# mburger-stsci/nexoclom

Hardware: AMD Instinct MI355X
Metric: particle*steps/s (higher is better)
Workload: dtype f64

## Files before the change

nexoclom_amd/csrc/nxc_device.hpp:

```cpp
#pragma once
#include <hip/hip_runtime.h>
#include <stdint.h>
#include "nxc_math.hpp"

struct LutDesc {
    int rec, fs, cell;
    int top;
    int last;
    int pad_;
    double xbase;
    double inv_w;
};
typedef LutDesc LutView;

extern __shared__ __align__(32) unsigned char nxc_lds[];

#define NXC_LDS_AS __attribute__((address_space(3)))
#define NXC_GLOBAL_AS __attribute__((address_space(1)))
typedef double nxc_v2d __attribute__((ext_vector_type(2)));

NXC_DEV double lds_f64(int byte_off)
{
    return *(const NXC_LDS_AS double *)(unsigned)byte_off;
}
// ... 491 lines not shown
    const double rn = nxc_sqrt((x * x + y * y) + z * z);
    const double en = nxc_sqrt(y * y + x * x);
    const double n0 = -z * x, n1 = -z * y, n2 = x * x + y * y;
    const double nn = nxc_sqrt((n0 * n0 + n1 * n1) + n2 * n2);
    const double dx = (v_t0 * (n0 / nn) + v_t1 * (y / en)) + v_rad * (x / rn);
    const double dy = (v_t0 * (n1 / nn) + v_t1 * (-x / en)) + v_rad * (y / rn);
    const double dz = (v_t0 * (n2 / nn) + v_t1 * 0.0) + v_rad * (z / rn);
    const double lonhit = fmod(atan2(x, -y) + TWO_PI, TWO_PI);
    const double lathit = asin(z);
    double tsurf = B.t0;
    if (lonhit <= 1.5707963267948966 || lonhit >= 4.71238898038469)
        tsurf = B.t0 + B.t1 * nxc_sqrt(nxc_sqrt(__builtin_fabs(cos(lonhit) * cos(lathit))));
    double v_new;
    if (B.accom == 0.0) {
        v_new = nxc_sqrt(v_old2);
    } else {
        const double v_emit = bispev3(B, tsurf, u_p) / B.unit_km;
        v_new = nxc_sqrt(v_emit * v_emit * B.accom + v_old2 * (1 - B.accom));
    }
    const double wx = dx * v_new, wy = dy * v_new, wz = dz * v_new;
    double frac = s[7];
    if (B.temp_dependent == 2) {
        double st = stick_map_at(B, lonhit, lathit);
        st = st > 1. ? 1. : (st < 0. ? 0. : st);
        frac *= (1 - st);
    } else if (B.temp_dependent) {
        double st = B.A0 * exp(B.A1 * tsurf) + B.A2;
        st = st > 1. ? 1. : (st < 0. ? 0. : st);
        frac *= (1 - st);
    } else if (B.stickcoef > 0) {
        frac *= (1 - B.stickcoef);
    }
    const double zero = ((x * 0.0 + y * 0.0) + (z * 0.0 + frac * 0.0)) + ((wx * 0.0 + wy * 0.0) + wz * 0.0);
    if (zero != 0.0) return false;
    s[1] = x; s[2] = y; s[3] = z;
    s[4] = wx; s[5] = wy; s[6] = wz;
    s[7] = frac;
    return true;
}

template <bool BOUNCE, bool NBODY = false>
NXC_DEV void apply_fate(double (&s)[8], double edge2, unsigned long long id, int &nbounce,
                        unsigned long long &nonfinite, const BodyK *Bd = nullptr,
                        const double *__restrict__ base = nullptr)
{
    const double r2 = (s[1] * s[1] + s[2] * s[2]) + s[3] * s[3];
    if (r2 < 1.0) {
        if (BOUNCE) {
            if (!bounce_packet(lds_header().B, s, r2, id, nbounce)) { s[7] = 0.0; nonfinite++; }
        } else s[7] = 0.0;
    }
    if (r2 > edge2) s[7] = 0.0;
    if (NBODY) {
        for (int m = 0; m < Bd->n_moons; m++) {
            double mx, my;
            moon_position(*Bd, base, m, 5, mx, my);
            const double dx = s[1] - mx, dy = s[2] - my;
            if ((dx * dx + dy * dy) + s[3] * s[3] < Bd->rad2[m]) s[7] = 0.0;
        }
    }
    if (s[7] < 1e-10) s[7] = 0.0;
    if (s[7] == 0.0) s[0] = 0.0;
}


NXC_DEV double wave_uniform(double v)
{
    const long long b = __double_as_longlong(v);
    const int lo = __builtin_amdgcn_readfirstlane((int)(b & 0xffffffffll));
    const int hi = __builtin_amdgcn_readfirstlane((int)(b >> 32));
    return __longlong_as_double(((long long)hi << 32) | (unsigned int)lo);
}
NXC_DEV int wave_uniform(int v) { return __builtin_amdgcn_readfirstlane(v); }

struct ImageRegs {
    double vrplanet;
    double x_lo, x_hi, x_inv_step, z_lo, z_hi, z_inv_step;
    int xedges, zedges, nx, nz, quantity, n_lines, downcast, dbg, x_is_x;
};

NXC_DEV ImageRegs image_regs(const ImageK &G)
{
    ImageRegs R;
    R.vrplanet = G.vrplanet;
    R.xedges = (int)G.xedges_off; R.zedges = (int)G.zedges_off;
    R.nx = G.nx; R.nz = G.nz;
    R.x_lo = lds_f64(R.xedges); R.x_hi = lds_f64(R.xedges + 8 * R.nx);
    R.z_lo = lds_f64(R.zedges); R.z_hi = lds_f64(R.zedges + 8 * R.nz);
    R.x_inv_step = G.x_inv_step; R.z_inv_step = G.z_inv_step;
    R.quantity = G.quantity; R.n_lines = G.n_lines; R.downcast = G.downcast_f32;
    R.x_is_x = wave_uniform(G.x_is_x);
#ifdef NXC_EXPERIMENT_KNOBS
    R.dbg = G.dbg;
#else
    R.dbg = 0;
#endif
    R.vrplanet = wave_uniform(R.vrplanet);
    R.x_lo = wave_uniform(R.x_lo); R.x_hi = wave_uniform(R.x_hi);
    R.z_lo = wave_uniform(R.z_lo); R.z_hi = wave_uniform(R.z_hi);
    R.x_inv_step = wave_uniform(R.x_inv_step); R.z_inv_step = wave_uniform(R.z_inv_step);
    R.xedges = wave_uniform(R.xedges); R.zedges = wave_uniform(R.zedges);
    R.nx = wave_uniform(R.nx); R.nz = wave_uniform(R.nz);
    R.quantity = wave_uniform(R.quantity); R.n_lines = wave_uniform(R.n_lines);
    R.downcast = wave_uniform(R.downcast);
#ifdef NXC_EXPERIMENT_KNOBS
    R.dbg = wave_uniform(R.dbg);
#endif
    return R;
}

NXC_DEV double nxc_div_const(double n, double d, double y)
{
    if (!((nxc_mid_range(n) || n == 0.0) && y == y)) return n / d;
    return nxc_div_seeded(n, d, y);
}

NXC_DEV int bin_index(double v, int edges, int n, double lo, double hi, double inv_step)
{
    if (!(v >= lo) || !(v <= hi)) return -1;
    int k = (int)((v - lo) * inv_step);
    k = k > n - 1 ? n - 1 : k;
    const double e0 = lds_f64(edges + 8 * k), e1 = lds_f64(edges + 8 * k + 8);
    if (__builtin_expect(!((v >= e0) && (v < e1)), 0)) {
        while (k > 0 && v < lds_f64(edges + 8 * k)) --k;
        while (k < n - 1 && v >= lds_f64(edges + 8 * (k + 1))) ++k;
    }
    return k;
}

NXC_DEV double f32_round_trip(double v) { return (double)(float)v; }

NXC_DEV int half_swap(int v, bool upper)
{
    const auto r = __builtin_amdgcn_permlane32_swap(v, v, false, false);
    return upper ? (int)r[0] : (int)r[1];
}

NXC_DEV void image_add_pairs(bool has, int pix, double w, double *__restrict__ acc2)
{
    if (__ballot(has) == 0) return;
    const bool upper = (threadIdx.x & 32) != 0;
    const int ppix = half_swap(has ? pix : -1, upper);
    const bool own = has && w != 0.0;
    const bool partner = ppix >= 0;
    {
        const bool act = upper ? partner : own;
        if (act)
            unsafeAtomicAdd(&acc2[2ll * (upper ? ppix : pix) + (upper ? 1 : 0)], upper ? 1.0 : w);
    }
    {
        const bool act = upper ? own : partner;
        if (act)
            unsafeAtomicAdd(&acc2[2ll * (upper ? pix : ppix) + (upper ? 0 : 1)], upper ? w : 1.0);
    }
}

NXC_DEV bool image_locate_core_xz(const ImageK &G, const ImageRegs &R, double x, double y, double z,
                                  double vy, double frac, double &radvel_out, double &fw_out,
                                  unsigned long long &nonfinite, int &ix_out, int &iz_out)
{
    const double radvel = vy + R.vrplanet;
    double xo, yo, zo;
    if (R.x_is_x) {
        xo = x;
        yo = G.M[4] * y + G.M[5] * z;
        zo = G.M[7] * y + G.M[8] * z;
    } else {
        xo = (G.M[0] * x + G.M[1] * y) + G.M[2] * z;
        yo = (G.M[3] * x + G.M[4] * y) + G.M[5] * z;
        zo = (G.M[6] * x + G.M[7] * y) + G.M[8] * z;
    }
    const int ix = bin_index(xo, R.xedges, R.nx, R.x_lo, R.x_hi, R.x_inv_step);
    const int iz = bin_index(zo, R.zedges, R.nz, R.z_lo, R.z_hi, R.z_inv_step);
    if (ix < 0 || iz < 0) {
        if (!(__builtin_fabs(frac) <= 1.7976931348623157e308) || radvel != radvel) nonfinite++;
        return false;
    }
    const double s_obs = xo * xo + zo * zo;
    const bool inview = (s_obs > 0x1.0000000000001p+0) || (yo < 0.0);
    frac = inview ? frac : frac * 0.0;
    if (R.quantity != 0)
        frac = sunlit(x, y, z) ? frac : frac * 0.0;
    radvel_out = radvel;
    fw_out = frac;
    ix_out = ix; iz_out = iz;
    return true;
}

NXC_DEV int image_locate_core(const ImageK &G, const ImageRegs &R, double x, double y, double z,
                              double vy, double frac, double &radvel_out, double &fw_out,
                              unsigned long long &nonfinite)
{
    int ix = 0, iz = 0;
    if (!image_locate_core_xz(G, R, x, y, z, vy, frac, radvel_out, fw_out, nonfinite, ix, iz))
        return -1;
    return ix * R.nz + iz;
}

NXC_DEV int image_locate(const ImageK &G, const ImageRegs &R, double x, double y, double z,
                         double vy, double frac, double &radvel_out, double &fw_out,
                         unsigned long long &nonfinite)
{
    if (R.downcast) {
        x = f32_round_trip(x); y = f32_round_trip(y); z = f32_round_trip(z);
        vy = f32_round_trip(vy); frac = f32_round_trip(frac);
    }
    return image_locate_core(G, R, x, y, z, vy, frac, radvel_out, fw_out, nonfinite);
}

NXC_DEV bool image_frame_test(const ImageK &G, const ImageRegs &R, double x, double y, double z,
                              double vy, double frac, float &xf, float &yf, float &zf,
                              unsigned long long &nonfinite)
{
    xf = (float)x; yf = (float)y; zf = (float)z;
    const double xd = xf, yd = yf, zd = zf;
    double xo, zo;
    if (R.x_is_x) {
        xo = xd;
        zo = G.M[7] * yd + G.M[8] * zd;
    } else {
        xo = (G.M[0] * xd + G.M[1] * yd) + G.M[2] * zd;
        zo = (G.M[6] * xd + G.M[7] * yd) + G.M[8] * zd;
    }
    const bool inside = (xo >= R.x_lo) && (xo <= R.x_hi) && (zo >= R.z_lo) && (zo <= R.z_hi);
    if (!inside && (!(__builtin_fabs(frac) < 0x1.ffffffp127) || vy != vy)) nonfinite++;
    return inside;
}

NXC_DEV bool image_weight(const ImageK &G, const ImageRegs &R, double radvel, double fw,
                          double &w_out)
{
    double w = fw;
    if (R.quantity != 0) {
        double gg = 0.0;
        if (R.n_lines == 2) {
            const LutView v0 = lut_view(G.line[0]), v1 = lut_view(G.line[1]);
            LutProbe p0, p1;
            lut_probe_cell(v0, radvel, p0); lut_probe_cell(v1, radvel, p1);
            lut_probe_rows(v0, p0); lut_probe_rows(v1, p1);
            const double g0 = lut_finish(v0, p0);
            gg = g0 + lut_finish(v1, p1);
        } else {
            gg = R.n_lines > 0 ? lut_interp(lut_view(G.line[0]), radvel) : 0.0;
#pragma unroll
            for (int l = 1; l < 4; l++)
                if (l < R.n_lines) gg += lut_interp(lut_view(G.line[l]), radvel);
        }
        w = nxc_div_const(fw * gg, 1e6, lds_header().Wt.rs_1e6);
    }
    w = nxc_div_const(w, G.apix_cm2, lds_header().Wt.rs_apix);
    w_out = w;
    return (__builtin_fabs(w) <= 1.7976931348623157e308) && radvel == radvel;
}

NXC_DEV void image_sample(const ImageK &G, const ImageRegs &R, bool has, double x, double y,
                          double z, double vy, double frac, double *__restrict__ acc2,
                          unsigned long long &binned, unsigned long long &nonfinite)
{
    int pix = -1;
    double radvel = 0.0, fw = 0.0, w = 0.0;
    if (has) pix = image_locate(G, R, x, y, z, vy, frac, radvel, fw, nonfinite);
    bool ok = pix >= 0;
    if (ok && !image_weight(G, R, radvel, fw, w)) { nonfinite++; ok = false; }
    binned += ok;
    image_add_pairs(ok, pix, w, acc2);
}

constexpr int NXC_IMGQ_SLOTS = 128;
constexpr int NXC_IMGQ_BYTES = NXC_IMGQ_SLOTS * (8 + 8 + 4);

struct ImageQueue {
    int head = 0, tail = 0;

    NXC_DEV void push(bool has, int pix, double radvel, double fw, int qoff)
    {
        const unsigned long long m = __ballot(has);
        if (m == 0) return;
        if (has) {
            const int lane = threadIdx.x & 63;
            const int slot = (tail + __popcll(m & ((1ull << lane) - 1ull))) & (NXC_IMGQ_SLOTS - 1);
            *reinterpret_cast<double *>(nxc_lds + qoff + 8 * slot) = radvel;
            *reinterpret_cast<double *>(nxc_lds + qoff + 8 * NXC_IMGQ_SLOTS + 8 * slot) = fw;
            *reinterpret_cast<int *>(nxc_lds + qoff + 16 * NXC_IMGQ_SLOTS + 4 * slot) = pix;
        }
        tail += __popcll(m);
        __builtin_amdgcn_fence(__ATOMIC_RELEASE, "wavefront");
        __builtin_amdgcn_wave_barrier();
    }
    NXC_DEV void push_sample(bool has, float x, float y, float z, float vy, float frac, int qoff)
    {
        const unsigned long long m = __ballot(has);
        if (m == 0) return;
        if (has) {
            const int lane = threadIdx.x & 63;
            const int slot = (tail + __popcll(m & ((1ull << lane) - 1ull))) & (NXC_IMGQ_SLOTS - 1);
            float *q = reinterpret_cast<float *>(nxc_lds + qoff) + slot;
            q[0] = x; q[NXC_IMGQ_SLOTS] = y; q[2 * NXC_IMGQ_SLOTS] = z;
            q[3 * NXC_IMGQ_SLOTS] = vy; q[4 * NXC_IMGQ_SLOTS] = frac;
        }
        tail += __popcll(m);
        __builtin_amdgcn_fence(__ATOMIC_RELEASE, "wavefront");
        __builtin_amdgcn_wave_barrier();
    }
    NXC_DEV bool pop_sample(int qoff, double &x, double &y, double &z, double &vy, double &frac)
    {
        __builtin_amdgcn_fence(__ATOMIC_ACQUIRE, "wavefront");
        const int n = waiting() < 64 ? waiting() : 64;
        const int lane = threadIdx.x & 63;
        const bool mine = lane < n;
        if (mine) {
            const int slot = (head + lane) & (NXC_IMGQ_SLOTS - 1);
            const float *q = reinterpret_cast<const float *>(nxc_lds + qoff) + slot;
            x = q[0]; y = q[NXC_IMGQ_SLOTS]; z = q[2 * NXC_IMGQ_SLOTS];
            vy = q[3 * NXC_IMGQ_SLOTS]; frac = q[4 * NXC_IMGQ_SLOTS];
        }
        head += n;
        __builtin_amdgcn_wave_barrier();
        return mine;
    }
    NXC_DEV int waiting() const { return tail - head; }
    NXC_DEV bool pop(int qoff, int &pix, double &radvel, double &fw)
    {
        __builtin_amdgcn_fence(__ATOMIC_ACQUIRE, "wavefront");
        const int n = waiting() < 64 ? waiting() : 64;
        const int lane = threadIdx.x & 63;
        const bool mine = lane < n;
        if (mine) {
            const int slot = (head + lane) & (NXC_IMGQ_SLOTS - 1);
            radvel = *reinterpret_cast<const double *>(nxc_lds + qoff + 8 * slot);
            fw = *reinterpret_cast<const double *>(nxc_lds + qoff + 8 * NXC_IMGQ_SLOTS + 8 * slot);
            pix = *reinterpret_cast<const int *>(nxc_lds + qoff + 16 * NXC_IMGQ_SLOTS + 4 * slot);
        }
        head += n;
        __builtin_amdgcn_wave_barrier();
        return mine;
    }
};
```

nexoclom_amd/csrc/nxc_kernels.hpp:

```cpp
#pragma once
#include "nxc_device.hpp"

struct DevCounters {
    unsigned long long particle_steps, samples, samples_binned, nonfinite, bad_step, neg_frac,
        unfinished, queue_head;
    unsigned long long wave_trips;
#ifdef NXC_STAMPS
    unsigned long long stamp[8];
#endif
};

#ifdef NXC_STAMPS
NXC_DEV unsigned long long nxc_stamp()
{
    unsigned long long t;
    __builtin_amdgcn_sched_barrier(0);
    asm volatile("s_memtime %0\n\ts_waitcnt lgkmcnt(0)" : "=s"(t) : : "memory");
    __builtin_amdgcn_sched_barrier(0);
    return t;
}
#define NXC_STAMP(k) do { const unsigned long long t_ = nxc_stamp(); seg[k] += t_ - t_prev; t_prev = t_; } while (0)
#else
#define NXC_STAMP(k) do { } while (0)
#endif

constexpr int NXC_BLOCK = 256;
#ifndef NXC_BLOCK_PERSIST_N
#define NXC_BLOCK_PERSIST_N 768
#endif
#ifndef NXC_CHUNK_N
#define NXC_CHUNK_N 32
#endif
constexpr int NXC_BLOCK_PERSIST = NXC_BLOCK_PERSIST_N;
constexpr int NXC_CHUNK = NXC_CHUNK_N;
static_assert(NXC_CHUNK >= 1 && NXC_CHUNK <= 64, "a chunk is loaded by one wave");
constexpr int NXC_WAVE_STAGE_BYTES = NXC_CHUNK * 9 * 8;
constexpr int NXC_WAVE_LDS_BYTES = NXC_WAVE_STAGE_BYTES + NXC_IMGQ_BYTES;
constexpr int NXC_WAVE_LDS_BYTES_ROWS = NXC_CHUNK * 11 * 8;

NXC_DEV void stage_tables(const unsigned char *__restrict__ blob, int64_t bytes)
{
    if ((unsigned)(size_t)(NXC_LDS_AS unsigned char *)nxc_lds != 0u) __builtin_trap();
    const unsigned long long *src = reinterpret_cast<const unsigned long long *>(blob);
    unsigned long long *dst = reinterpret_cast<unsigned long long *>(nxc_lds);
    const int64_t words = bytes >> 3;
    for (int64_t w = threadIdx.x; w < words; w += blockDim.x) dst[w] = src[w];
    __syncthreads();
    if (threadIdx.x == 0) {
        LdsHeader &H = lds_header_rw();
        H.Wt.rs_1e6 = nxc_recip_seed(1e6);
        H.Wt.rs_apix = nxc_mid_range(H.G.apix_cm2) ? nxc_recip_seed(H.G.apix_cm2)
                                                   : __builtin_nan("");
    }
    __syncthreads();
}

NXC_DEV void stage_tables_and_args(const unsigned char *__restrict__ blob, int64_t bytes,
                                   const double *soa0, const unsigned *order, double *final_out,
                                   long long *steps_out, unsigned long long *head, long long n,
                                   const long long *offsets = nullptr,
                                   const unsigned long long *avail = nullptr)
{
    stage_tables(blob, bytes);
    if (threadIdx.x == 0) {
        LoopK &L = lds_header_rw().L;
        L.soa0 = soa0; L.order = order; L.final_out = final_out; L.steps_out = steps_out;
        L.head = head; L.n = n; L.offsets = offsets; L.avail = avail;
        L.q_rec = order ? 8 : 1; L.q_col = order ? 1 : n;
    }
    __syncthreads();
}

NXC_DEV unsigned long long wave_sum(unsigned long long v)
{
#pragma unroll
    for (int off = 32; off > 0; off >>= 1) v += __shfl_down(v, off, 64);
    return v;
}

NXC_DEV void flush_counter(unsigned long long *dst, unsigned long long v)
{
    v = wave_sum(v);
    if ((threadIdx.x & 63) == 0 && v) atomicAdd(dst, v);
}

NXC_DEV void flush_counters_wg(unsigned long long *lds, unsigned long long *d0, unsigned long long v0,
                               unsigned long long *d1, unsigned long long v1,
                               unsigned long long *d2, unsigned long long v2)
{
    __syncthreads();
    if (threadIdx.x < 3) lds[threadIdx.x] = 0ull;
    __syncthreads();
    v0 = wave_sum(v0); v1 = wave_sum(v1); v2 = wave_sum(v2);
    if ((threadIdx.x & 63) == 0) {
        if (v0) atomicAdd(&lds[0], v0);
        if (v1) atomicAdd(&lds[1], v1);
        if (v2) atomicAdd(&lds[2], v2);
    }
    __syncthreads();
    if (threadIdx.x == 0) {
        if (lds[0]) atomicAdd(d0, lds[0]);
        if (lds[1]) atomicAdd(d1, lds[1]);
        if (lds[2]) atomicAdd(d2, lds[2]);
    }
}

NXC_DEV long long wave_bcast0(long long v)
{
    int lo = __builtin_amdgcn_readfirstlane((int)(v & 0xffffffffll));
    int hi = __builtin_amdgcn_readfirstlane((int)(v >> 32));
    return ((long long)hi << 32) | (unsigned int)lo;
}

__global__ void __launch_bounds__(NXC_BLOCK)
k_state(ForceK F, const unsigned char *__restrict__ blob, int64_t stage_bytes, int64_t n,
        const double *__restrict__ x, const double *__restrict__ y, const double *__restrict__ z,
        const double *__restrict__ vy, double *__restrict__ ax, double *__restrict__ ay,
        double *__restrict__ az, double *__restrict__ ion)
{
    stage_tables(blob, stage_bytes);
    const LutView T = lut_view(F.tab);
    for (int64_t i = (int64_t)blockIdx.x * blockDim.x + threadIdx.x; i < n;
         i += (int64_t)gridDim.x * blockDim.x) {
        double a0, a1, a2, l;
        state_eval<false>(F, T, x[i], y[i], z[i], vy[i], a0, a1, a2, l);
        ax[i] = a0; ay[i] = a1; az[i] = a2; ion[i] = l;
    }
}

template <bool DELTA>
__global__ void __launch_bounds__(NXC_BLOCK)
k_rk5_step(ForceK F, const unsigned char *__restrict__ blob, int64_t stage_bytes, int64_t n,
           const double *__restrict__ in, const double *__restrict__ hstep,
           double *__restrict__ out, double *__restrict__ delta)
{
    stage_tables(blob, stage_bytes);
    const LutView T = lut_view(F.tab);
    for (int64_t i = (int64_t)blockIdx.x * blockDim.x + threadIdx.x; i < n;
         i += (int64_t)gridDim.x * blockDim.x) {
        double s[8], d[8];
#pragma unroll
        for (int c = 0; c < 8; c++) s[c] = in[c * n + i];
        rk5_step<DELTA, false>(F, T, s, hstep[i], StepW{}, d);
#pragma unroll
        for (int c = 0; c < 8; c++) out[c * n + i] = s[c];
        if (DELTA) {
#pragma unroll
            for (int c = 0; c < 8; c++) delta[c * n + i] = d[c];
        }
    }
}

constexpr int NXC_REC_DOUBLES = 10;
constexpr int NXC_REC_FLOATS = 10;
typedef float nxc_v4f __attribute__((ext_vector_type(4)));
typedef float nxc_v2f __attribute__((ext_vector_type(2)));
typedef float nxc_v4f_a8 __attribute__((ext_vector_type(4), aligned(8)));

template <int ROWS>
NXC_DEV void store_record(void *__restrict__ rec, long long row, const double (&s)[8],
                          double lossfrac, long long id)
{
    if (ROWS == 2) {
        float *p = static_cast<float *>(rec) + row * NXC_REC_FLOATS;
        nxc_v4f a, b;
        nxc_v2f c;
        a.x = (float)s[0]; a.y = (float)s[1]; a.z = (float)s[2]; a.w = (float)s[3];
        b.x = (float)s[4]; b.y = (float)s[5]; b.z = (float)s[6]; b.w = (float)s[7];
        c.x = (float)lossfrac; c.y = __int_as_float((int)id);
        *reinterpret_cast<nxc_v4f_a8 *>(p) = a;
        *reinterpret_cast<nxc_v4f_a8 *>(p + 4) = b;
        *reinterpret_cast<nxc_v2f *>(p + 8) = c;
    } else {
        nxc_v2d *p = reinterpret_cast<nxc_v2d *>(static_cast<double *>(rec) + row * NXC_REC_DOUBLES);
        nxc_v2d a, b, c, d, e;
        a.x = s[0]; a.y = s[1]; b.x = s[2]; b.y = s[3]; c.x = s[4]; c.y = s[5]; d.x = s[6]; d.y = s[7];
        e.x = lossfrac; e.y = __longlong_as_double(id);
        p[0] = a; p[1] = b; p[2] = c; p[3] = d; p[4] = e;
    }
}

constexpr int NXC_TR_ROWS = 256;
template <typename T, typename I>
__global__ void __launch_bounds__(NXC_TR_ROWS)
k_rows_transpose(const void *__restrict__ rec_, long long total, T *__restrict__ cols,
                 I *__restrict__ index)
{
    static_assert(sizeof(T) == sizeof(I), "a record is ten equal-sized slots");
    typedef T pair_t __attribute__((ext_vector_type(2)));
    __shared__ pair_t tile[NXC_TR_ROWS * 5];
    const T *rec = static_cast<const T *>(rec_);
    for (long long base = (long long)blockIdx.x * NXC_TR_ROWS; base < total;
         base += (long long)gridDim.x * NXC_TR_ROWS) {
        const int nrow = (int)((total - base) < NXC_TR_ROWS ? (total - base) : NXC_TR_ROWS);
        const pair_t *src = reinterpret_cast<const pair_t *>(rec + base * 10);
        for (int w = threadIdx.x; w < nrow * 5; w += NXC_TR_ROWS) tile[w] = src[w];
        __syncthreads();
        if ((int)threadIdx.x < nrow) {
            const T *r = reinterpret_cast<const T *>(tile) + threadIdx.x * 10;
            const long long row = base + threadIdx.x;
#pragma unroll
            for (int c = 0; c < 9; c++) cols[c * total + row] = r[c];
            I id;
            __builtin_memcpy(&id, &r[9], sizeof id);
            index[row] = id;
        }
        __syncthreads();
    }
}

constexpr int NXC_DENSIFY_RECORDS = 32;
__global__ void __launch_bounds__(NXC_BLOCK)
k_rows_densify(const double *__restrict__ rec, const long long *__restrict__ offsets,
               const double *__restrict__ final_soa, const long long *__restrict__ steps,
               int64_t n, int64_t nrec, double *__restrict__ traj)
{
    const int64_t i = (int64_t)blockIdx.x * blockDim.x + threadIdx.x;
    if (i >= n) return;
    const long long off = offsets[i], len = offsets[i + 1] - off, last = steps[i];
    const int64_t k0 = (int64_t)blockIdx.y * NXC_DENSIFY_RECORDS;
    const int64_t k1 = k0 + NXC_DENSIFY_RECORDS < nrec ? k0 + NXC_DENSIFY_RECORDS : nrec;
    for (int64_t k = k0; k < k1; k++) {
        double v[8] = {0, 0, 0, 0, 0, 0, 0, 0};
        if (k < len) {
            const nxc_v2d *r = reinterpret_cast<const nxc_v2d *>(rec + (off + k) * NXC_REC_DOUBLES);
#pragma unroll
            for (int c = 0; c < 4; c++) { const nxc_v2d t = r[c]; v[2 * c] = t.x; v[2 * c + 1] = t.y; }
        } else if (k == last) {
#pragma unroll
            for (int c = 0; c < 8; c++) v[c] = final_soa[c * n + i];
        }
#pragma unroll
        for (int c = 0; c < 8; c++) traj[((int64_t)c * nrec + k) * n + i] = v[c];
    }
}

NXC_DEV bool wait_published(const unsigned long long *avail, unsigned long long need)
{
    unsigned long long t0 = 0;
    bool timing = false;
    for (;;) {
        const unsigned long long v =
            __hip_atomic_load(avail, __ATOMIC_ACQUIRE, __HIP_MEMORY_SCOPE_AGENT);
        if (v == ~0ull) return false;
        if (v >= need) return true;
        const unsigned long long now = __builtin_amdgcn_s_memrealtime();
        if (!timing) { t0 = now; timing = true; }
        else if (now - t0 > 300000000ull) return false;
        __builtin_amdgcn_s_sleep(32);
    }
}

__global__ void k_publish(unsigned long long *avail, unsigned long long value)
{
    if (threadIdx.x == 0 && blockIdx.x == 0)
        __hip_atomic_store(avail, value, __ATOMIC_RELEASE, __HIP_MEMORY_SCOPE_AGENT);
}

struct WaveQueue {
    long long pending = 0;
    int c_pos = 0, c_cnt = 0;
    bool drained = false, stalled = false;

    static NXC_DEV long long claim(unsigned long long *head)
    {
        return (long long)__hip_atomic_fetch_add((NXC_GLOBAL_AS unsigned long long *)head,
                                                 (unsigned long long)NXC_CHUNK, __ATOMIC_RELAXED,
                                                 __HIP_MEMORY_SCOPE_AGENT);
    }

    NXC_DEV void start()
    {
        if ((threadIdx.x & 63) == 0) pending = claim(lds_header().L.head);
    }

    template <bool ROWS = false, bool STREAMED = false>
    NXC_DEV long long refill(bool need, int stage_off, double (&s)[8], long long *row0 = nullptr,
                             long long *nrow = nullptr)
    {
        const unsigned long long mask = __ballot(need);
        long long mine = -1;
        if (mask == 0 || drained) return mine;
        const int want = __popcll(mask);
        const int lane = threadIdx.x & 63;
        const int rank = __popcll(mask & ((1ull << lane) - 1ull));
        NXC_LDS_AS double *stage = (NXC_LDS_AS double *)(unsigned)stage_off;
        int served = 0;
        while (served < want) {
            if (c_pos >= c_cnt) {
                const LoopK &L = lds_header().L;
                const long long n = L.n;
                const double *__restrict__ soa0 = L.soa0;
                const unsigned *__restrict__ ids = L.order;
                const long long b = wave_bcast0(pending);
                if (b >= n) { drained = true; break; }
                c_cnt = (b + NXC_CHUNK <= n) ? NXC_CHUNK : (int)(n - b);
                c_pos = 0;
                if (STREAMED) {
                    if (!wait_published(L.avail, (unsigned long long)(b + c_cnt))) {
                        drained = true; stalled = true; c_cnt = 0;
                        break;
                    }
                }
                __builtin_amdgcn_fence(__ATOMIC_RELEASE, "wavefront");
                if (lane < c_cnt) {
                    const long long q_col = L.q_col;
                    const NXC_GLOBAL_AS double *g = (const NXC_GLOBAL_AS double *)soa0 + (b + lane) * L.q_rec;
                    const NXC_GLOBAL_AS unsigned *gid = (const NXC_GLOBAL_AS unsigned *)ids;
                    double col[8];
#pragma unroll
                    for (int c = 0; c < 8; c++) col[c] = g[c * q_col];
                    const long long pid = gid ? (long long)gid[b + lane] : b + lane;
                    long long o0 = 0, o1 = 0;
                    if (ROWS) {
                        const NXC_GLOBAL_AS long long *offs = (const NXC_GLOBAL_AS long long *)L.offsets;
                        o0 = offs[pid]; o1 = offs[pid + 1];
                    }
#pragma unroll
                    for (int c = 0; c < 8; c++) stage[c * NXC_CHUNK + lane] = col[c];
                    stage[8 * NXC_CHUNK + lane] = __longlong_as_double(pid);
                    if (ROWS) {
                        stage[9 * NXC_CHUNK + lane] = __longlong_as_double(o0);
                        stage[10 * NXC_CHUNK + lane] = __longlong_as_double(o1 - o0);
                    }
                }
                if (lane == 0) pending = claim(L.head);
                __builtin_amdgcn_fence(__ATOMIC_ACQUIRE, "wavefront");
                __builtin_amdgcn_wave_barrier();
            }
            const int room = c_cnt - c_pos;
            const int take = room < (want - served) ? room : want - served;
            if (need && rank >= served && rank < served + take) {
                const int slot = c_pos + (rank - served);
                mine = __double_as_longlong(stage[8 * NXC_CHUNK + slot]);
#pragma unroll
                for (int c = 0; c < 8; c++) s[c] = stage[c * NXC_CHUNK + slot];
                if (ROWS) {
                    *row0 = __double_as_longlong(stage[9 * NXC_CHUNK + slot]);
                    *nrow = __double_as_longlong(stage[10 * NXC_CHUNK + slot]);
                }
            }
            c_pos += take;
            served += take;
        }
        return mine;
    }
};

template <int IMAGE>
NXC_DEV bool image_pop(ImageQueue &queue, int imgq_off, const ImageRegs &IR, int &p, double &rv,
                       double &fw, unsigned long long &nonfinite)
{
    if (IMAGE == 2) {
        double x = 0, y = 0, z = 0, vy = 0, frac = 0;
        const bool ok = queue.pop_sample(imgq_off, x, y, z, vy, frac);
        if (ok) p = image_locate_core(lds_header().G, IR, x, y, z, vy, frac, rv, fw, nonfinite);
        return ok && p >= 0;
    }
    return queue.pop(imgq_off, p, rv, fw);
}

template <int IMAGE, bool BOUNCE, bool FULL, bool NBODY = false, int ROWS = 0, bool STREAMED = false>
__global__ void __launch_bounds__(NXC_BLOCK_PERSIST)
k_const_fused(ForceK F, const unsigned char *__restrict__ blob,
              int64_t stage_bytes, int64_t n, const double *__restrict__ soa0,
              const unsigned *__restrict__ order, int64_t first_id, int64_t n_iter,
              double edge2, double *__restrict__ final_out,
              long long *__restrict__ steps_out, double *__restrict__ acc2,
              DevCounters *__restrict__ ctr, const double *__restrict__ moon_pos = nullptr,
              const long long *__restrict__ offsets = nullptr, void *__restrict__ rec = nullptr,
              const unsigned long long *__restrict__ avail = nullptr)
{
    static_assert(!(IMAGE && ROWS), "the rows pass has no image");
    static_assert(!(STREAMED && (ROWS || BOUNCE || NBODY)), "the streamed pass is the plain one");
    stage_tables_and_args(blob, stage_bytes, soa0, order, final_out, steps_out, &ctr->queue_head, n,
                          offsets, STREAMED ? avail : nullptr);
    const LutView T = lut_view(F.tab);
    ImageRegs IR{};
    if (IMAGE) IR = image_regs(lds_header().G);
    ImageQueue queue;
    unsigned my_steps = 0, my_samples = 0, my_binned = 0;
    unsigned long long my_nonfinite = 0;
    WaveQueue q;
    q.start();
    const bool want_out = __builtin_amdgcn_readfirstlane(
        (final_out != nullptr || steps_out != nullptr) ? 1 : 0) != 0;
    const int wave_off = (int)((stage_bytes + 31) & ~31ll) +
                         (threadIdx.x >> 6) * (ROWS ? NXC_WAVE_LDS_BYTES_ROWS : NXC_WAVE_LDS_BYTES);
    const int stage_off = wave_off, imgq_off = wave_off + NXC_WAVE_STAGE_BYTES;
    bool has = false, fresh = false;
    long long id = -1, row0 = 0, nrow = 0;
    double lossfrac = 0.0;
    unsigned my_overrun = 0, my_trips = 0;
    int k = 0, nbounce = 0;
    const int n_it = n_iter > 0x7fffffffll ? 0x7fffffff : (int)n_iter;
    double s[8], d[8];
#ifdef NXC_STAMPS
    unsigned long long seg[8] = {0, 0, 0, 0, 0, 0, 0, 0}, t_prev = nxc_stamp();
#endif
    for (;;) {
#ifdef NXC_REFILL_MIN
        const unsigned long long free_ = __ballot(!has);
        const bool serve = __popcll(free_) >= NXC_REFILL_MIN || free_ == ~0ull;
        const long long got = serve ? q.refill<ROWS != 0, STREAMED>(!has, stage_off, s, &row0, &nrow) : -1;
#else
        const long long got = q.refill<ROWS != 0, STREAMED>(!has, stage_off, s, &row0, &nrow);
#endif
        if (got >= 0) { id = got; k = 0; has = true; fresh = true; nbounce = 0; lossfrac = 0.0; }
        if (__ballot(has) == 0) break;
        my_trips++;
        NXC_STAMP(0);
        int p = -1;
        double rv = 0.0, fw = 0.0;
        bool inframe = false;
        float qx = 0.f, qy = 0.f, qz = 0.f;
        if (has) {
            const double before = s[7];
            if (!fresh) {
                if (NBODY) {
                    const BodyK *Bd = &lds_header().Bd;
                    const double *mp = moon_pos + (long long)k * (2 * Bd->n_moons);
                    rk5_step<false, true, FULL, true>(F, T, s, 0.0, lds_header().W, d, Bd, mp);
                    apply_fate<false, true>(s, edge2, 0ull, nbounce, my_nonfinite, Bd, mp);
                } else {
                    rk5_step<false, true, FULL>(F, T, s, 0.0, lds_header().W, d);
                    apply_fate<BOUNCE>(s, edge2, (unsigned long long)(first_id + id), nbounce, my_nonfinite);
                }
#ifdef NXC_PROBE_VMOV
                {
                    int junk;
#pragma unroll
                    for (int j = 0; j < NXC_PROBE_VMOV; j++) asm volatile("v_mov_b32 %0, 0x12345" : "=v"(junk));
                }
#endif
#ifdef NXC_PROBE_FMA
                {
                    double j0 = s[1], j1 = s[2], j2 = s[3], j3 = s[4];
#pragma unroll
                    for (int j = 0; j < NXC_PROBE_FMA / 4; j++) {
                        asm volatile("v_fma_f64 %0, %0, %0, %0" : "+v"(j0));
                        asm volatile("v_fma_f64 %0, %0, %0, %0" : "+v"(j1));
                        asm volatile("v_fma_f64 %0, %0, %0, %0" : "+v"(j2));
                        asm volatile("v_fma_f64 %0, %0, %0, %0" : "+v"(j3));
                    }
                }
#endif
                k++; my_steps++;
                if (ROWS) lossfrac = (lossfrac + before) - s[7];
            }
            NXC_STAMP(1);
            fresh = false;
            const bool live = s[7] > 0.0;
            if (ROWS && live) {
                if (k < nrow) store_record<ROWS>(rec, row0 + k, s, lossfrac, id);
                else my_overrun++;
            }
            if (IMAGE && live) {
                my_samples++;
                if (IMAGE == 2)
                    inframe = image_frame_test(lds_header().G, IR, s[1], s[2], s[3], s[5], s[7], qx,
                                               qy, qz, my_nonfinite);
                else
                    p = image_locate(lds_header().G, IR, s[1], s[2], s[3], s[5], s[7], rv, fw,
                                     my_nonfinite);
            }
            NXC_STAMP(2);
            if (!live || k >= n_it) {
                if (want_out) {
                    const LoopK &L = lds_header().L;
                    if (NXC_GLOBAL_AS double *fo = (NXC_GLOBAL_AS double *)L.final_out) {
                        const long long np = L.n;
#pragma unroll
                        for (int c = 0; c < 8; c++) fo[c * np + id] = s[c];
                    }
                    if (NXC_GLOBAL_AS long long *so = (NXC_GLOBAL_AS long long *)L.steps_out) so[id] = k;
                }
                has = false;
            }
        }
        NXC_STAMP(3);
        if (IMAGE) {
#ifdef NXC_EXPERIMENT_KNOBS
            if (IR.dbg == 3) { my_binned += IMAGE == 2 ? inframe : p >= 0; continue; }
#endif
            if (IMAGE == 2) queue.push_sample(inframe, qx, qy, qz, (float)s[5], (float)s[7], imgq_off);
            else queue.push(p >= 0, p, rv, fw, imgq_off);
            NXC_STAMP(4);
            if (queue.waiting() >= 64) {
                double w = 0.0;
                bool ok = image_pop<IMAGE>(queue, imgq_off, IR, p, rv, fw, my_nonfinite);
#ifdef NXC_EXPERIMENT_KNOBS
                if (IR.dbg == 2) { my_binned += ok; continue; }
#endif
                if (ok && !image_weight(lds_header().G, IR, rv, fw, w)) { my_nonfinite++; ok = false; }
                my_binned += ok;
                NXC_STAMP(5);
#ifdef NXC_EXPERIMENT_KNOBS
                if (IR.dbg == 1) { my_nonfinite += (w == 12345.678); continue; }
#endif
                image_add_pairs(ok, p, w, acc2);
                NXC_STAMP(6);
            }
        }
    }
#ifdef NXC_STAMPS
    if ((threadIdx.x & 63) == 0)
        for (int c = 0; c < 8; c++) atomicAdd(&ctr->stamp[c], seg[c]);
#endif
    if (IMAGE) {
        while (queue.waiting() > 0) {
            int p = -1;
            double rv = 0.0, fw = 0.0, w = 0.0;
            bool ok = image_pop<IMAGE>(queue, imgq_off, IR, p, rv, fw, my_nonfinite);
            if (ok && !image_weight(lds_header().G, IR, rv, fw, w)) { my_nonfinite++; ok = false; }
            my_binned += ok;
            image_add_pairs(ok, p, w, acc2);
        }
    }
    flush_counter(&ctr->particle_steps, my_steps);
    if ((threadIdx.x & 63) == 0) atomicAdd(&ctr->wave_trips, (unsigned long long)my_trips);
    if (ROWS) flush_counter(&ctr->unfinished, my_overrun);
    if (STREAMED && q.stalled && (threadIdx.x & 63) == 0) atomicAdd(&ctr->unfinished, 1ull);
    if (IMAGE) {
        flush_counter(&ctr->samples, my_samples);
        flush_counter(&ctr->samples_binned, my_binned);
    }
    if (IMAGE || BOUNCE) flush_counter(&ctr->nonfinite, my_nonfinite);
}

#ifdef NXC_VAR_TRACE
__device__ unsigned long long g_var_trace[8 * 4096];
#endif
#ifndef NXC_VAR_FAIR
#define NXC_VAR_FAIR 1
#endif
#ifndef NXC_VAR_MERGE_MAX_N
#define NXC_VAR_MERGE_MAX_N 48
#endif
#ifndef NXC_VAR_PRIO_SHIFT
#define NXC_VAR_PRIO_SHIFT 12
#endif
constexpr int NXC_VAR_MERGE_MAX = NXC_VAR_MERGE_MAX_N;
constexpr int NXC_VAR_HDR_OFF = NXC_WAVE_LDS_BYTES - 64;
constexpr unsigned NXC_VAR_PENDING = 0xffffffffu;
static_assert(NXC_VAR_MERGE_MAX * 11 * 8 <= NXC_VAR_HDR_OFF && NXC_VAR_HDR_OFF >= NXC_WAVE_STAGE_BYTES,
              "a donor's packets and the header share the wave's block with the staging area");
struct VarMerge {
    int wave0;
    NXC_DEV NXC_LDS_AS double *seg(int w) const
    {
        return (NXC_LDS_AS double *)(unsigned)(wave0 + w * NXC_WAVE_LDS_BYTES);
    }
    NXC_DEV NXC_LDS_AS unsigned *hdr(int w) const
    {
        return (NXC_LDS_AS unsigned *)(unsigned)(wave0 + w * NXC_WAVE_LDS_BYTES + NXC_VAR_HDR_OFF);
    }
    NXC_DEV NXC_LDS_AS int *room(int k) const { return (NXC_LDS_AS int *)(hdr(0) + 4 + k); }
    NXC_DEV static unsigned ld(NXC_LDS_AS unsigned *a)
    {
        return __hip_atomic_load(a, __ATOMIC_ACQUIRE, __HIP_MEMORY_SCOPE_WORKGROUP);
    }
    NXC_DEV void publish(int w, unsigned count) const
    {
        __hip_atomic_store(hdr(w), count, __ATOMIC_RELEASE, __HIP_MEMORY_SCOPE_WORKGROUP);
    }
};

template <bool FULL, bool FAIR_>
__global__ void __launch_bounds__(NXC_BLOCK_PERSIST)
k_var(ForceK F, const unsigned char *__restrict__ blob, int64_t stage_bytes, int64_t n,
      const double *__restrict__ soa0, const unsigned *__restrict__ order, double resolution, double outeredge, long long max_steps,
      double *__restrict__ final_out, double *__restrict__ hstore_out,
      DevCounters *__restrict__ ctr)
{
    constexpr bool FAIR = FAIR_ && NXC_VAR_FAIR;
    const int wave = threadIdx.x >> 6, lane = threadIdx.x & 63;
    const int nw = blockDim.x >> 6;
    const VarMerge M{(int)((stage_bytes + 31) & ~31ll)};
    if (FAIR && lane == 0) {
        M.hdr(wave)[0] = NXC_VAR_PENDING; M.hdr(wave)[1] = 0u; M.hdr(wave)[2] = 0u;
        if (wave == 0)
            for (int k = 4; k < 12; k++) M.hdr(0)[k] = 0u;
    }
    stage_tables_and_args(blob, stage_bytes, soa0, order, final_out, nullptr, &ctr->queue_head, n);
    bool keeper = false, published = false, settled = false;
    int prev_live = -1, prio = 0;
    auto hw_simd = []() { return (int)__builtin_amdgcn_s_getreg((1 << 11) | (4 << 6) | 4); };
    auto hw_slot = []() { return (int)__builtin_amdgcn_s_getreg((3 << 11) | (0 << 6) | 4); };
    if (FAIR) {
        const int simd = hw_simd();
        unsigned r = 0;
        if (lane == 0) r = __hip_atomic_fetch_add(M.hdr(0) + 8 + simd, 1u, __ATOMIC_RELAXED, __HIP_MEMORY_SCOPE_WORKGROUP);
        keeper = __builtin_amdgcn_readfirstlane(r) == 0;
        if (keeper && lane == 0) M.publish(wave, 0u);
    }
    const LutView T = lut_view(F.tab);
    const double resx = resolution, resv = 0.1 * resolution, resf = resolution;
    unsigned long long my_steps = 0, my_nonfinite = 0, my_bad = 0, my_neg = 0, my_unfinished = 0;
    WaveQueue q;
    q.start();
    const int stage_off = M.wave0 + wave * NXC_WAVE_LDS_BYTES;
    bool has = false;
    long long id = -1, it = 0;
    unsigned my_trips = 0;
    double s[8], hs = 1000.0;
#ifdef NXC_VAR_TRACE
    const unsigned long long tr_start = __builtin_amdgcn_s_memrealtime();
    unsigned long long tr_drain = 0, tr_low = 0;
    unsigned tr_trips_drain = 0, tr_trips_low = 0;
#endif
    for (;;) {
        const long long got = q.refill(!has, stage_off, s);
#ifdef NXC_VAR_TRACE
        if (q.drained && tr_drain == 0) { tr_drain = __builtin_amdgcn_s_memrealtime(); tr_trips_drain = my_trips; }
        if (q.drained && tr_low == 0 && __popcll(__ballot(has)) <= 8) { tr_low = __builtin_amdgcn_s_memrealtime(); tr_trips_low = my_trips; }
#endif
        if (got >= 0) {
            id = got; it = 0; hs = 1000.0; has = true;
        }
        if (FAIR && q.drained && !settled) {
            const int simd = hw_simd();
            const unsigned long long livem = __ballot(has);
            int live = __popcll(livem);
            if (!keeper) {
                if (live > 0 && live <= NXC_VAR_MERGE_MAX) {
                    int r = 0;
                    if (lane < 4) r = __hip_atomic_load(M.room(lane), __ATOMIC_RELAXED, __HIP_MEMORY_SCOPE_WORKGROUP);
                    const unsigned long long can = __ballot(lane < 4 && r >= live);
                    if (can != 0) {
                        const int k = (can >> simd) & 1ull ? simd : (int)__builtin_ctzll(can);
                        int old = 0;
                        if (lane == 0) {
                            old = __hip_atomic_fetch_sub(M.room(k), live, __ATOMIC_RELAXED, __HIP_MEMORY_SCOPE_WORKGROUP);
                            if (old < live) __hip_atomic_fetch_add(M.room(k), live, __ATOMIC_RELAXED, __HIP_MEMORY_SCOPE_WORKGROUP);
                        }
                        if (__builtin_amdgcn_readfirstlane(old) >= live) {
                            if (has) {
                                NXC_LDS_AS double *e = M.seg(wave) + __popcll(livem & ((1ull << lane) - 1ull));
#pragma unroll
                                for (int c = 0; c < 8; c++) e[c * NXC_VAR_MERGE_MAX] = s[c];
                                e[8 * NXC_VAR_MERGE_MAX] = hs;
                                e[9 * NXC_VAR_MERGE_MAX] = __longlong_as_double(it);
                                e[10 * NXC_VAR_MERGE_MAX] = __longlong_as_double(id);
                                has = false;
                            }
                            if (lane == 0) { M.hdr(wave)[1] = (unsigned)k; M.publish(wave, (unsigned)live); }
                            published = true;
                        }
                    }
                }
            } else {
                const int freed = prev_live < 0 ? 64 - live : prev_live - live;
                if (freed > 0 && lane == 0)
                    __hip_atomic_fetch_add(M.room(simd), freed, __ATOMIC_RELAXED, __HIP_MEMORY_SCOPE_WORKGROUP);
                bool mine = false;
                unsigned c = 0;
                if (lane < nw) {
                    c = M.ld(M.hdr(lane));
                    mine = c != NXC_VAR_PENDING && c != 0u && M.hdr(lane)[1] == (unsigned)simd && M.hdr(lane)[2] == 0u;
                }
                unsigned long long offer = __ballot(mine);
                if (offer == 0 && __ballot(lane < nw && c == NXC_VAR_PENDING) == 0) {
                    settled = true;
                    __builtin_amdgcn_s_setprio(0);
                }
                while (offer != 0) {
                    const int w = __builtin_ctzll(offer);
                    offer &= offer - 1;
                    const int got = __shfl((int)c, w, 64);
                    const unsigned long long freem = __ballot(!has);
                    const int rank = __popcll(freem & ((1ull << lane) - 1ull));
                    if (!has && rank < got) {
                        const NXC_LDS_AS double *e = M.seg(w) + rank;
#pragma unroll
                        for (int c2 = 0; c2 < 8; c2++) s[c2] = e[c2 * NXC_VAR_MERGE_MAX];
                        hs = e[8 * NXC_VAR_MERGE_MAX];
                        it = __double_as_longlong(e[9 * NXC_VAR_MERGE_MAX]);
                        id = __double_as_longlong(e[10 * NXC_VAR_MERGE_MAX]);
                        has = true;
                    }
                    if (lane == 0) M.hdr(w)[2] = 1u;
                    live += got;
                }
                prev_live = live;
            }
        }
        if (__ballot(has) == 0) {
            if (!FAIR || !keeper || settled) break;
            const int simd = hw_simd();
            bool open = false;
            if (lane < nw) {
                const unsigned c = M.ld(M.hdr(lane));
                open = c == NXC_VAR_PENDING || (c != 0u && M.hdr(lane)[1] == (unsigned)simd && M.hdr(lane)[2] == 0u);
            }
            if (__ballot(open) == 0) break;
            __builtin_amdgcn_s_sleep(8);
            continue;
        }
        my_trips++;
        if (FAIR && !settled && (my_trips & 3u) == 0) {
            const unsigned long long t = __builtin_amdgcn_s_memrealtime();
            const int pr = (int)(((t >> NXC_VAR_PRIO_SHIFT) + (unsigned long long)hw_slot()) % 3ull);
            if (pr != prio) {
                prio = pr;
                if (pr == 2) __builtin_amdgcn_s_setprio(2);
                else if (pr == 1) __builtin_amdgcn_s_setprio(1);
                else __builtin_amdgcn_s_setprio(0);
            }
        }
        if (has) {
            bool done = !(s[0] > resolution && s[7] > 0.0);
            if (!done && it >= max_steps) { my_unfinished++; done = true; }
            if (!done) {
                const double h = __builtin_fmin(s[0], hs);
                if (!(h > 0.0)) { my_bad++; done = true; }
                else {
                    double t[8], d[8];
#pragma unroll
                    for (int c = 0; c < 8; c++) t[c] = s[c];
                    rk5_step<true, false, FULL>(F, T, t, h, StepW{}, d);
                    my_steps++; it++;
                    const double fscale = resf + __builtin_fabs(t[7]) * resf;
                    double e = d[0];
                    bool finite = true;
#pragma unroll
                    for (int c = 1; c <= 7; c++) {
                        const double scale = c <= 3 ? resx + __builtin_fabs(t[c]) * resx
                                           : c <= 6 ? resv + __builtin_fabs(t[c]) * resv : fscale;
                        const double q = nxc_div(d[c], scale);
                        finite = finite && (__builtin_fabs(q) <= 1.7976931348623157e308);
                        e = __builtin_fmax(e, q);
                    }
                    if (!finite) e = __builtin_nan("");
                    if (!(__builtin_fabs(e) <= 1.7976931348623157e308)) { my_nonfinite++; done = true; }
                    else {
                        if (t[7] < 0.0 && e < 1.0) my_neg++;
                        if ((t[7] - s[7] > fscale) && (e > 1.0)) e = 1.1;
                        double hold = h;
                        if (e < 1e-7) { e = 1.0; hold = h * 10; }
                        if (e < 1.0) {
                            { int nb_ = 0; apply_fate<false>(t, outeredge, 0ull, nb_, my_nonfinite); }
#pragma unroll
                            for (int c = 0; c < 8; c++) s[c] = t[c];
                        } else {
                            const double hn = 0.95 * hold * nxc_pow_m025(e);
                            if (!(__builtin_fabs(hn) <= 1.7976931348623157e308)) { my_bad++; done = true; }
                            else hs = __builtin_fmax(hn, 0.1 * hold);
                        }
                    }
                }
            }
            if (done) {
#pragma unroll
                for (int c = 0; c < 8; c++) final_out[c * n + id] = s[c];
#ifdef NXC_VAR_TRACE
                if (hstore_out) hstore_out[id] = (double)it;
#else
                if (hstore_out) hstore_out[id] = hs;
#endif
                has = false;
            }
        }
    }
    if (FAIR && !keeper && !published && lane == 0) M.publish(wave, 0u);
#ifdef NXC_VAR_TRACE
    if ((threadIdx.x & 63) == 0) {
        const unsigned hw = __builtin_amdgcn_s_getreg((5 << 11) | (0 << 6) | 4);
        unsigned long long *tr = g_var_trace + 8 * ((blockIdx.x * (blockDim.x >> 6) + (threadIdx.x >> 6)) & 4095);
        tr[0] = tr_start; tr[1] = tr_drain; tr[2] = tr_low; tr[3] = __builtin_amdgcn_s_memrealtime();
        tr[4] = my_trips; tr[5] = tr_trips_drain; tr[6] = tr_trips_low; tr[7] = hw;
    }
#endif
    flush_counter(&ctr->particle_steps, my_steps);
    if ((threadIdx.x & 63) == 0) atomicAdd(&ctr->wave_trips, (unsigned long long)my_trips);
    flush_counter(&ctr->nonfinite, my_nonfinite);
    flush_counter(&ctr->bad_step, my_bad);
    flush_counter(&ctr->neg_frac, my_neg);
    flush_counter(&ctr->unfinished, my_unfinished);
}

constexpr int NXC_IMAGE_BLOCK = 1024;
template <typename T>
__global__ void __launch_bounds__(NXC_IMAGE_BLOCK)
k_image(const unsigned char *__restrict__ blob, int64_t stage_bytes, int64_t p,
        const T *__restrict__ x, const T *__restrict__ y, const T *__restrict__ z,
        const T *__restrict__ vy, const T *__restrict__ frac,
        double *__restrict__ acc2, DevCounters *__restrict__ ctr)
{
    stage_tables(blob, stage_bytes);
    const ImageRegs IR = image_regs(lds_header().G);
    unsigned long long my_samples = 0, my_binned = 0, my_nonfinite = 0;
    for (int64_t base = (int64_t)blockIdx.x * blockDim.x; base < p;
         base += (int64_t)gridDim.x * blockDim.x) {
        const int64_t i = base + threadIdx.x;
        const bool has = i < p;
        my_samples += has;
        double sx = 0, sy = 0, sz = 0, svy = 0, sf = 0;
        if (has) { sx = x[i]; sy = y[i]; sz = z[i]; svy = vy[i]; sf = frac[i]; }
        image_sample(lds_header().G, IR, has, sx, sy, sz, svy, sf, acc2, my_binned, my_nonfinite);
    }
    flush_counters_wg(reinterpret_cast<unsigned long long *>(nxc_lds), &ctr->samples, my_samples,
                      &ctr->samples_binned, my_binned, &ctr->nonfinite, my_nonfinite);
}

// ... 1722 lines not shown
```

Measured before the change: 33.40 billion.

## Issue refill and image-queue LDS reads before the RK step to hide latency

Splits the wave-queue refill and the image-queue pop into an issue phase and a later consume phase. For the FULL, non-bounce, non-nbody, non-streamed variant, the LDS/global reads for new particles and queued samples now start before the RK5 step, and their results are consumed after it, so memory latency overlaps with compute. Newly served particles land in a shadow buffer and are copied into the state afterwards, which replaces the old 'fresh' flag. This adds register pressure from the shadow state and the held image slot, and it reorders the drain relative to the push.

```diff
diff --git a/nexoclom_amd/csrc/nxc_device.hpp b/nexoclom_amd/csrc/nxc_device.hpp
--- a/nexoclom_amd/csrc/nxc_device.hpp
+++ b/nexoclom_amd/csrc/nxc_device.hpp
@@ -817,7 +817,7 @@
         __builtin_amdgcn_fence(__ATOMIC_RELEASE, "wavefront");
         __builtin_amdgcn_wave_barrier();
     }
-    NXC_DEV bool pop_sample(int qoff, double &x, double &y, double &z, double &vy, double &frac)
+    NXC_DEV bool pop_sample_issue(int qoff, float (&v)[5])
     {
         __builtin_amdgcn_fence(__ATOMIC_ACQUIRE, "wavefront");
         const int n = waiting() < 64 ? waiting() : 64;
@@ -826,8 +826,8 @@
         if (mine) {
             const int slot = (head + lane) & (NXC_IMGQ_SLOTS - 1);
             const float *q = reinterpret_cast<const float *>(nxc_lds + qoff) + slot;
-            x = q[0]; y = q[NXC_IMGQ_SLOTS]; z = q[2 * NXC_IMGQ_SLOTS];
-            vy = q[3 * NXC_IMGQ_SLOTS]; frac = q[4 * NXC_IMGQ_SLOTS];
+#pragma unroll
+            for (int c = 0; c < 5; c++) v[c] = q[c * NXC_IMGQ_SLOTS];
         }
         head += n;
         __builtin_amdgcn_wave_barrier();
diff --git a/nexoclom_amd/csrc/nxc_kernels.hpp b/nexoclom_amd/csrc/nxc_kernels.hpp
--- a/nexoclom_amd/csrc/nxc_kernels.hpp
+++ b/nexoclom_amd/csrc/nxc_kernels.hpp
@@ -275,11 +275,11 @@
     }
 
     template <bool ROWS = false, bool STREAMED = false>
-    NXC_DEV long long refill(bool need, int stage_off, double (&s)[8], long long *row0 = nullptr,
-                             long long *nrow = nullptr)
+    NXC_DEV bool refill_issue(bool need, int stage_off, double (&t)[8], long long &tid,
+                              long long *trow0 = nullptr, long long *tnrow = nullptr)
     {
         const unsigned long long mask = __ballot(need);
-        long long mine = -1;
+        bool mine = false;
         if (mask == 0 || drained) return mine;
         const int want = __popcll(mask);
         const int lane = threadIdx.x & 63;
@@ -290,8 +290,6 @@
             if (c_pos >= c_cnt) {
                 const LoopK &L = lds_header().L;
                 const long long n = L.n;
-                const double *__restrict__ soa0 = L.soa0;
-                const unsigned *__restrict__ ids = L.order;
                 const long long b = wave_bcast0(pending);
                 if (b >= n) { drained = true; break; }
                 c_cnt = (b + NXC_CHUNK <= n) ? NXC_CHUNK : (int)(n - b);
@@ -305,8 +303,8 @@
                 __builtin_amdgcn_fence(__ATOMIC_RELEASE, "wavefront");
                 if (lane < c_cnt) {
                     const long long q_col = L.q_col;
-                    const NXC_GLOBAL_AS double *g = (const NXC_GLOBAL_AS double *)soa0 + (b + lane) * L.q_rec;
-                    const NXC_GLOBAL_AS unsigned *gid = (const NXC_GLOBAL_AS unsigned *)ids;
+                    const NXC_GLOBAL_AS double *g = (const NXC_GLOBAL_AS double *)L.soa0 + (b + lane) * L.q_rec;
+                    const NXC_GLOBAL_AS unsigned *gid = (const NXC_GLOBAL_AS unsigned *)L.order;
                     double col[8];
 #pragma unroll
                     for (int c = 0; c < 8; c++) col[c] = g[c * q_col];
@@ -332,12 +330,13 @@
             const int take = room < (want - served) ? room : want - served;
             if (need && rank >= served && rank < served + take) {
                 const int slot = c_pos + (rank - served);
-                mine = __double_as_longlong(stage[8 * NXC_CHUNK + slot]);
-#pragma unroll
-                for (int c = 0; c < 8; c++) s[c] = stage[c * NXC_CHUNK + slot];
+                mine = true;
+                tid = __double_as_longlong(stage[8 * NXC_CHUNK + slot]);
+#pragma unroll
+                for (int c = 0; c < 8; c++) t[c] = stage[c * NXC_CHUNK + slot];
                 if (ROWS) {
-                    *row0 = __double_as_longlong(stage[9 * NXC_CHUNK + slot]);
-                    *nrow = __double_as_longlong(stage[10 * NXC_CHUNK + slot]);
+                    *trow0 = __double_as_longlong(stage[9 * NXC_CHUNK + slot]);
+                    *tnrow = __double_as_longlong(stage[10 * NXC_CHUNK + slot]);
                 }
             }
             c_pos += take;
@@ -345,19 +344,65 @@
         }
         return mine;
     }
+
+    static NXC_DEV void refill_take(bool served, const double (&t)[8], double (&s)[8])
+    {
+        if (served) {
+#pragma unroll
+            for (int c = 0; c < 8; c++) s[c] = t[c];
+        }
+    }
+
+    NXC_DEV long long refill(bool need, int stage_off, double (&s)[8])
+    {
+        long long id = -1;
+        return refill_issue(need, stage_off, s, id) ? id : -1;
+    }
 };
+
+struct ImageSlot {
+    float f[5] = {0.f, 0.f, 0.f, 0.f, 0.f};
+    int pix = -1;
+    double rv = 0.0, fw = 0.0;
+};
+
+template <int IMAGE>
+NXC_DEV void image_slot_settle(const ImageSlot &v)
+{
+    if (IMAGE == 2)
+        asm volatile("" :: "v"(v.f[0]), "v"(v.f[1]), "v"(v.f[2]), "v"(v.f[3]), "v"(v.f[4]));
+    else
+        asm volatile("" :: "v"(v.pix), "v"(v.rv), "v"(v.fw));
+}
+
+template <int IMAGE>
+NXC_DEV bool image_pop_issue(ImageQueue &queue, int imgq_off, ImageSlot &v)
+{
+    if (IMAGE == 2) return queue.pop_sample_issue(imgq_off, v.f);
+    return queue.pop(imgq_off, v.pix, v.rv, v.fw);
+}
+
+template <int IMAGE>
+NXC_DEV bool image_pop_finish(bool ok, const ImageSlot &v, const ImageRegs &IR, int &p, double &rv,
+                              double &fw, unsigned long long &nonfinite)
+{
+    if (IMAGE == 2) {
+        if (ok) p = image_locate_core(lds_header().G, IR, (double)v.f[0], (double)v.f[1],
+                                      (double)v.f[2], (double)v.f[3], (double)v.f[4], rv, fw,
+                                      nonfinite);
+        return ok && p >= 0;
+    }
+    if (ok) { p = v.pix; rv = v.rv; fw = v.fw; }
+    return ok;
+}
 
 template <int IMAGE>
 NXC_DEV bool image_pop(ImageQueue &queue, int imgq_off, const ImageRegs &IR, int &p, double &rv,
                        double &fw, unsigned long long &nonfinite)
 {
-    if (IMAGE == 2) {
-        double x = 0, y = 0, z = 0, vy = 0, frac = 0;
-        const bool ok = queue.pop_sample(imgq_off, x, y, z, vy, frac);
-        if (ok) p = image_locate_core(lds_header().G, IR, x, y, z, vy, frac, rv, fw, nonfinite);
-        return ok && p >= 0;
-    }
-    return queue.pop(imgq_off, p, rv, fw);
+    ImageSlot v;
+    const bool ok = image_pop_issue<IMAGE>(queue, imgq_off, v);
+    return image_pop_finish<IMAGE>(ok, v, IR, p, rv, fw, nonfinite);
 }
 
 template <int IMAGE, bool BOUNCE, bool FULL, bool NBODY = false, int ROWS = 0, bool STREAMED = false>
@@ -388,68 +433,87 @@
     const int wave_off = (int)((stage_bytes + 31) & ~31ll) +
                          (threadIdx.x >> 6) * (ROWS ? NXC_WAVE_LDS_BYTES_ROWS : NXC_WAVE_LDS_BYTES);
     const int stage_off = wave_off, imgq_off = wave_off + NXC_WAVE_STAGE_BYTES;
-    bool has = false, fresh = false;
+    bool has = false;
     long long id = -1, row0 = 0, nrow = 0;
     double lossfrac = 0.0;
     unsigned my_overrun = 0, my_trips = 0;
     int k = 0, nbounce = 0;
     const int n_it = n_iter > 0x7fffffffll ? 0x7fffffff : (int)n_iter;
     double s[8], d[8];
+    constexpr bool EARLY = FULL && !BOUNCE && !NBODY && !STREAMED;
 #ifdef NXC_STAMPS
     unsigned long long seg[8] = {0, 0, 0, 0, 0, 0, 0, 0}, t_prev = nxc_stamp();
 #endif
+    ImageSlot slot;
     for (;;) {
+        double shadow[8];
+        double (&t)[8] = *(EARLY ? &shadow : &s);
+        long long tid = -1, trow0 = 0, tnrow = 0;
 #ifdef NXC_REFILL_MIN
         const unsigned long long free_ = __ballot(!has);
         const bool serve = __popcll(free_) >= NXC_REFILL_MIN || free_ == ~0ull;
-        const long long got = serve ? q.refill<ROWS != 0, STREAMED>(!has, stage_off, s, &row0, &nrow) : -1;
+        const bool served = serve && q.refill_issue<ROWS != 0, STREAMED>(!has, stage_off, t, tid, &trow0, &tnrow);
 #else
-        const long long got = q.refill<ROWS != 0, STREAMED>(!has, stage_off, s, &row0, &nrow);
-#endif
-        if (got >= 0) { id = got; k = 0; has = true; fresh = true; nbounce = 0; lossfrac = 0.0; }
-        if (__ballot(has) == 0) break;
+        const bool served = q.refill_issue<ROWS != 0, STREAMED>(!has, stage_off, t, tid, &trow0, &tnrow);
+#endif
+        auto take = [&]() {
+            WaveQueue::refill_take(served, t, s);
+            if (served) {
+                id = tid; k = 0; has = true; nbounce = 0; lossfrac = 0.0;
+                if (ROWS) { row0 = trow0; nrow = tnrow; }
+            }
+        };
+        if (!EARLY) take();
+        if (__ballot(has || served) == 0) break;
         my_trips++;
+        bool drain = false, popped = false;
+        if (IMAGE && EARLY) {
+            drain = queue.waiting() >= 64;
+            if (drain) popped = image_pop_issue<IMAGE>(queue, imgq_off, slot);
+        }
         NXC_STAMP(0);
+        if (has && !served) {
+            const double before = s[7];
+            if (NBODY) {
+                const BodyK *Bd = &lds_header().Bd;
+                const double *mp = moon_pos + (long long)k * (2 * Bd->n_moons);
+                rk5_step<false, true, FULL, true>(F, T, s, 0.0, lds_header().W, d, Bd, mp);
+                apply_fate<false, true>(s, edge2, 0ull, nbounce, my_nonfinite, Bd, mp);
+            } else {
+                rk5_step<false, true, FULL>(F, T, s, 0.0, lds_header().W, d);
+                apply_fate<BOUNCE>(s, edge2, (unsigned long long)(first_id + id), nbounce, my_nonfinite);
+            }
+#ifdef NXC_PROBE_VMOV
+            {
+                int junk;
+#pragma unroll
+                for (int j = 0; j < NXC_PROBE_VMOV; j++) asm volatile("v_mov_b32 %0, 0x12345" : "=v"(junk));
+            }
+#endif
+#ifdef NXC_PROBE_FMA
+            {
+                double j0 = s[1], j1 = s[2], j2 = s[3], j3 = s[4];
+#pragma unroll
+                for (int j = 0; j < NXC_PROBE_FMA / 4; j++) {
+                    asm volatile("v_fma_f64 %0, %0, %0, %0" : "+v"(j0));
+                    asm volatile("v_fma_f64 %0, %0, %0, %0" : "+v"(j1));
+                    asm volatile("v_fma_f64 %0, %0, %0, %0" : "+v"(j2));
+                    asm volatile("v_fma_f64 %0, %0, %0, %0" : "+v"(j3));
+                }
+            }
+#endif
+            k++; my_steps++;
+            if (ROWS) lossfrac = (lossfrac + before) - s[7];
+        }
+        if (IMAGE && EARLY) image_slot_settle<IMAGE>(slot);
+        NXC_STAMP(1);
+        if (EARLY) take();
+        NXC_STAMP(7);
         int p = -1;
         double rv = 0.0, fw = 0.0;
         bool inframe = false;
         float qx = 0.f, qy = 0.f, qz = 0.f;
         if (has) {
-            const double before = s[7];
-            if (!fresh) {
-                if (NBODY) {
-                    const BodyK *Bd = &lds_header().Bd;
-                    const double *mp = moon_pos + (long long)k * (2 * Bd->n_moons);
-                    rk5_step<false, true, FULL, true>(F, T, s, 0.0, lds_header().W, d, Bd, mp);
-                    apply_fate<false, true>(s, edge2, 0ull, nbounce, my_nonfinite, Bd, mp);
-                } else {
-                    rk5_step<false, true, FULL>(F, T, s, 0.0, lds_header().W, d);
-                    apply_fate<BOUNCE>(s, edge2, (unsigned long long)(first_id + id), nbounce, my_nonfinite);
-                }
-#ifdef NXC_PROBE_VMOV
-                {
-                    int junk;
-#pragma unroll
-                    for (int j = 0; j < NXC_PROBE_VMOV; j++) asm volatile("v_mov_b32 %0, 0x12345" : "=v"(junk));
-                }
-#endif
-#ifdef NXC_PROBE_FMA
-                {
-                    double j0 = s[1], j1 = s[2], j2 = s[3], j3 = s[4];
-#pragma unroll
-                    for (int j = 0; j < NXC_PROBE_FMA / 4; j++) {
-                        asm volatile("v_fma_f64 %0, %0, %0, %0" : "+v"(j0));
-                        asm volatile("v_fma_f64 %0, %0, %0, %0" : "+v"(j1));
-                        asm volatile("v_fma_f64 %0, %0, %0, %0" : "+v"(j2));
-                        asm volatile("v_fma_f64 %0, %0, %0, %0" : "+v"(j3));
-                    }
-                }
-#endif
-                k++; my_steps++;
-                if (ROWS) lossfrac = (lossfrac + before) - s[7];
-            }
-            NXC_STAMP(1);
-            fresh = false;
             const bool live = s[7] > 0.0;
             if (ROWS && live) {
                 if (k < nrow) store_record<ROWS>(rec, row0 + k, s, lossfrac, id);
@@ -483,23 +547,32 @@
 #ifdef NXC_EXPERIMENT_KNOBS
             if (IR.dbg == 3) { my_binned += IMAGE == 2 ? inframe : p >= 0; continue; }
 #endif
+            auto weigh_and_add = [&]() {
+                int dp = -1;
+                double drv = 0.0, dfw = 0.0, w = 0.0;
+                bool ok = image_pop_finish<IMAGE>(popped, slot, IR, dp, drv, dfw, my_nonfinite);
+#ifdef NXC_EXPERIMENT_KNOBS
+                const int dbg = IR.dbg;
+#else
+                const int dbg = 0;
+#endif
+                if (dbg == 2) my_binned += ok;
+                else {
+                    if (ok && !image_weight(lds_header().G, IR, drv, dfw, w)) { my_nonfinite++; ok = false; }
+                    my_binned += ok;
+                    NXC_STAMP(5);
+                    if (dbg == 1) my_nonfinite += (w == 12345.678);
+                    else image_add_pairs(ok, dp, w, acc2);
+                    NXC_STAMP(6);
+                }
+            };
+            if (drain) weigh_and_add();
             if (IMAGE == 2) queue.push_sample(inframe, qx, qy, qz, (float)s[5], (float)s[7], imgq_off);
             else queue.push(p >= 0, p, rv, fw, imgq_off);
             NXC_STAMP(4);
-            if (queue.waiting() >= 64) {
-                double w = 0.0;
-                bool ok = image_pop<IMAGE>(queue, imgq_off, IR, p, rv, fw, my_nonfinite);
-#ifdef NXC_EXPERIMENT_KNOBS
-                if (IR.dbg == 2) { my_binned += ok; continue; }
-#endif
-                if (ok && !image_weight(lds_header().G, IR, rv, fw, w)) { my_nonfinite++; ok = false; }
-                my_binned += ok;
-                NXC_STAMP(5);
-#ifdef NXC_EXPERIMENT_KNOBS
-                if (IR.dbg == 1) { my_nonfinite += (w == 12345.678); continue; }
-#endif
-                image_add_pairs(ok, p, w, acc2);
-                NXC_STAMP(6);
+            if (!EARLY && queue.waiting() >= 64) {
+                popped = image_pop_issue<IMAGE>(queue, imgq_off, slot);
+                weigh_and_add();
             }
         }
     }
```

Result: slower. 32.98 billion (-1.3%).
